# ucla-vision/xivo

Measured on AMD Instinct MI355X. Metric: EKF updates/sec (state dim 250, 80 feats) @1 GPU; % MFMA roofline, higher is better.
Workload: dtype f64; 1 GPU; MH gating + UpdateJosephForm: state dim 250, 80 features (M=160), XIVO row sparsity, P/H/inn/R resident in HBM; filters_per_gpu=16384, global_batch=16384, parallelism=replicas x1 (no collective), pipeline=sparse-H (row-pair compressed H, whitened in-solve Joseph form), hand_over=dense H -> row-pair compressed rows every step, inside the timed region, route=sparse_in_solve, not_spd_filters=0

## Files before the change

### xivo_amd/csrc/chol_trsm.hip

```cpp
#include <stdlib.h>

#include "mfma_util.h"
#include <stdio.h>

#include "trsm_lds_kernel.h"

namespace xivo_hip {

namespace {

__global__ __launch_bounds__(256) void fwd_vec_kernel(const double* __restrict__ LUall, long strideLU, int ldlu,
                                                     const double* __restrict__ invDall, long strideInvD,
                                                     const double* __restrict__ innall, long strideInn, double* __restrict__ yall,
                                                     long strideY, int Mp, int batch) {
  __shared__ double sy[4][384];
  const int wv = threadIdx.x >> 6;
  const int filt = blockIdx.x * (blockDim.x >> 6) + wv;
  if (filt >= batch) return;
  const int lane = threadIdx.x & 63, r = lane & 15, part = lane >> 4;
  const double* L = LUall + (long)filt * strideLU;
  const double* invD = invDall + (long)filt * strideInvD;
  const double* inn = innall + (long)filt * strideInn;
  double* y = yall + (long)filt * strideY;
  double* ys = sy[wv];
  const int nb = Mp / 16;
  for (int k = 0; k < nb; ++k) {
    double acc = 0.0;
    for (int c = part; c < 16 * k; c += 4) acc = fma(L[(16 * k + r) + (long)c * ldlu], ys[c], acc);
    acc += __shfl_xor(acc, 16);
    acc += __shfl_xor(acc, 32);
    const double rhs = inn[16 * k + r] - acc;
    double out = 0.0;
#pragma unroll
    for (int c = 0; c < 16; ++c) out = fma(invD[(long)k * 512 + r + 16 * c], __shfl(rhs, c), out);
    if (part == 0) { ys[16 * k + r] = out; y[16 * k + r] = out; }
  }
}


template <int NBM>
__global__ __launch_bounds__(1024) void pnew_reg_f64_kernel(PnewRegArgs g) {
  extern __shared__ __attribute__((aligned(16))) double sL[];
  const int bidx = blockIdx.x;
  const int filt = (bidx >> 3) * 8 + (bidx & 7);
  if (filt >= g.batch) return;
  if (g.skip_status && g.skip_status[filt] != 0) return;
  const int tid = threadIdx.x, lane = tid & 63, wave = __builtin_amdgcn_readfirstlane(tid >> 6);
  const int li = lane & 15, lg = lane >> 4;
  const int nb = g.Mp / 16;
  const int c0 = wave * 16;
  const bool live = c0 < g.Np;
  const double* __restrict__ G = g.G + (long)filt * g.strideG;
  d4 X[NBM];
#pragma unroll
  for (int i = 0; i < NBM; ++i) {
    X[i] = d4{0.0, 0.0, 0.0, 0.0};
    if (live && i < nb) {
#pragma unroll
      for (int r = 0; r < 4; ++r) X[i][r] = G[(c0 + li) + (long)(16 * i + lg + 4 * r) * g.ldg];
    }
  }
  sym_tiles_from_regs<NBM>(X, X, sL, g.K + (long)filt * g.strideK, g.ldk, g.T + (long)filt * g.strideT, g.ldt,
                           g.P + (long)filt * g.strideP, g.ldp, nb, g.Np / 16, g.jbp, live, wave, wave, lane);
}

template <int NBM, int WH, int NWS = 8>
__global__ __launch_bounds__(64 * NWS, NWS == 8 ? (NBM <= 4 ? 6 : (NBM <= 8 ? 4 : 2)) : 2) void trsm_stream_f64_kernel(TrsmArgs g) {
  extern __shared__ __attribute__((aligned(16))) double sL[];
  constexpr int PSZ = (NBM + 1) * 256;
  constexpr int WCOLS = 16 * NWS;
  const int chunks = (g.Np + WCOLS - 1) / WCOLS;
  const int b = blockIdx.x;
  const int xcd = b & 7, slot = b >> 3;
  const int filt = (slot / chunks) * 8 + xcd;
  const int chunk = slot % chunks;
  if (filt >= g.batch) return;
  const int tid = threadIdx.x, lane = tid & 63, wave = __builtin_amdgcn_readfirstlane(tid >> 6);
  const int li = lane & 15, lg = lane >> 4;
  const int nb = g.Mp / 16;
  const double* __restrict__ LU = g.LU + (long)filt * g.strideLU;
  const double* __restrict__ invD = g.invD + (long)filt * g.strideInvD;
  const long ld = g.ldlu;
  const int c0 = chunk * WCOLS + wave * 16;
  const bool live = c0 < g.Np;
  const __amdgpu_buffer_rsrc_t rPHT = buf_rsrc(g.PHT + (long)filt * g.stridePHT), rK = buf_rsrc(g.K + (long)filt * g.strideK),
                               rInn = buf_rsrc(g.fwd_only ? g.y + (long)filt * g.strideY : g.inn + (long)filt * g.strideInn),
                               rY = buf_rsrc(WH ? g.Yout + (long)filt * g.strideY2 : g.K);
  const unsigned vPHT = (unsigned)((live ? c0 + li : 0) + lg * g.ldpht) * 8u;
  const unsigned vK = (unsigned)((live ? c0 + li : 0) + lg * g.ldk) * 8u;
  const unsigned vY = WH ? (unsigned)((live ? c0 + li : 0) + lg * g.ldy2) * 8u : 0u;

  d4 X[NBM];
#pragma unroll
  for (int i = 0; i < NBM; ++i) {
    X[i] = d4{0.0, 0.0, 0.0, 0.0};
    if (live && i < nb) {
#pragma unroll
      for (int r = 0; r < 4; ++r) X[i][r] = buf_ld(rPHT, vPHT, (unsigned)((16 * i + 4 * r) * g.ldpht) * 8u);
    }
  }

  auto issue_panel = [&](int k, bool fwd, double* buf) {
    const int j0 = fwd ? k : 0, nj = (fwd ? nb - k : k + 1) + ((WH && !fwd) ? 1 : 0);
    for (int q = wave; q < nj * 2; q += NWS) {
      int j = j0 + (q >> 1);
      const int h = q & 1;
      const bool extra = WH && !fwd && (q >> 1) == nj - 1;
      const double* src;
      if (extra) { j = nb; src = LU + (16 * k + 2 * (lane & 7)) + (long)(16 * k + 8 * h + (lane >> 3)) * ld; }
      else if (j == k) src = invD + (long)k * 512 + (fwd ? 0 : 256) + h * 128 + 2 * lane;
      else src = LU + (16 * j + 2 * (lane & 7)) + (long)(16 * k + 8 * h + (lane >> 3)) * ld;
      __builtin_amdgcn_global_load_lds((const __attribute__((address_space(1))) void*)src,
                                       (__attribute__((address_space(3))) void*)(buf + j * 256 + h * 128), 16, 0, 0);
    }
  };
  double* buf0 = sL;
  double* buf1 = sL + PSZ;

  issue_panel(0, true, buf0);
#pragma unroll
  for (int k = 0; k < NBM; ++k) {
    if (k < nb) {
      asm volatile("s_waitcnt vmcnt(0)" ::: "memory");
      __syncthreads();
      const double* cur = (k & 1) ? buf1 : buf0;
      if (k + 1 < nb) issue_panel(k + 1, true, (k & 1) ? buf0 : buf1);
      if (live) {
        d4 t = d4{0.0, 0.0, 0.0, 0.0};
#pragma unroll
        for (int s = 0; s < 4; ++s) t = mfma(cur[k * 256 + li + 16 * (4 * s + lg)], X[k][s], t);
        X[k] = t;
#pragma unroll
        for (int s = 0; s < 4; ++s) {
#pragma unroll
          for (int i = k + 1; i < NBM; ++i) {
            if (i < nb) X[i] = mfma(-cur[i * 256 + li + 16 * (4 * s + lg)], t[s], X[i]);
          }
        }
      }
      __builtin_amdgcn_sched_barrier(0);
    }
  }
  double part = 0.0;
  if (WH && live) {
#pragma unroll
    for (int i = 0; i < NBM; ++i) {
      if (i < nb) {
#pragma unroll
        for (int r = 0; r < 4; ++r) buf_st(X[i][r], rK, vK, (unsigned)((16 * i + 4 * r) * g.ldk) * 8u);
      }
      __builtin_amdgcn_sched_barrier(0);
    }
  }
  __syncthreads();
  if (!g.fwd_only) issue_panel(nb - 1, false, buf0);
  int par = 0;
#pragma unroll
  for (int k = NBM - 1; k >= 0; --k) {
    if (k < nb && !g.fwd_only) {
      asm volatile("s_waitcnt vmcnt(0)" ::: "memory");
      __syncthreads();
      const double* cur = par ? buf1 : buf0;
      if (k > 0) issue_panel(k - 1, false, par ? buf0 : buf1);
      par ^= 1;
      if (live) {
        d4 wk = d4{0.0, 0.0, 0.0, 0.0};
        if (WH) {
          if (k == nb - 1) wk = X[k];
          else {
#pragma unroll
            for (int r = 0; r < 4; ++r) wk[r] = buf_ld(rK, vK, (unsigned)((16 * k + 4 * r) * g.ldk) * 8u);
          }
        }
        d4 t = d4{0.0, 0.0, 0.0, 0.0};
#pragma unroll
        for (int s = 0; s < 4; ++s) t = mfma(cur[k * 256 + li + 16 * (4 * s + lg)], X[k][s], t);
        if (WH) {
#pragma unroll
          for (int s2 = 0; s2 < 4; ++s2) {
            const int kk = 4 * s2 + lg;
            const double a = cur[nb * 256 + li + 16 * kk];
            X[k] = mfma(kk >= li ? -a : 0.0, t[s2], X[k]);
          }
#pragma unroll
          for (int r = 0; r < 4; ++r) part = fma(t[r], buf_ld(rInn, (unsigned)lg * 8u, (unsigned)(16 * k + 4 * r) * 8u), part);
        } else {
          X[k] = t;
        }
#pragma unroll
        for (int s = 0; s < 4; ++s) {
#pragma unroll
          for (int i = 0; i < k; ++i) X[i] = mfma(-cur[i * 256 + li + 16 * (4 * s + lg)], t[s], X[i]);
        }
        if (WH) {
#pragma unroll
          for (int r = 0; r < 4; ++r) {
            if (g.out_f32) buf_st_f32((float)(wk[r] + X[k][r]), rY, vY >> 1, (unsigned)((16 * k + 4 * r) * g.ldy2) * 4u);
            else buf_st(wk[r] + X[k][r], rY, vY, (unsigned)((16 * k + 4 * r) * g.ldy2) * 8u);
          }
          X[k] = wk - X[k];
        }
      }
      __builtin_amdgcn_sched_barrier(0);
    }
  }
  if (!live) return;
#pragma unroll
  for (int i = 0; i < NBM; ++i) {
    if (i < nb) {
#pragma unroll
      for (int r = 0; r < 4; ++r) {
        if (WH && g.out_f32) buf_st_f32((float)X[i][r], rY, vY >> 1, (unsigned)(g.Np * g.Mp + (16 * i + 4 * r) * g.ldy2) * 4u);
        else buf_st(X[i][r], rK, vK, (unsigned)((16 * i + 4 * r) * g.ldk) * 8u);
        if (!WH) part = fma(X[i][r], buf_ld(rInn, (unsigned)lg * 8u, (unsigned)(16 * i + 4 * r) * 8u), part);
      }
    }
    __builtin_amdgcn_sched_barrier(0);
  }
  part += __shfl_xor(part, 16);
  part += __shfl_xor(part, 32);
  if (lg == 0) g.err[(long)filt * g.strideErr + c0 + li] = part;
}

template <int NBM, int WH, int NWS = 8>
int launch_trsm_stream_t(const TrsmArgs& g, hipStream_t stream) {
  const int chunks = (g.Np + 16 * NWS - 1) / (16 * NWS);
  const int grid = ((g.batch + 7) / 8) * 8 * chunks;
  const size_t lds = (size_t)2 * (NBM + 1) * 256 * sizeof(double);
  static bool attr_set = false;
  if (!attr_set) {
    (void)hipFuncSetAttribute(reinterpret_cast<const void*>(&trsm_stream_f64_kernel<NBM, WH, NWS>), hipFuncAttributeMaxDynamicSharedMemorySize, 160 * 1024);
    attr_set = true;
  }
  hipLaunchKernelGGL((trsm_stream_f64_kernel<NBM, WH, NWS>), dim3(grid), dim3(64 * NWS), lds, stream, g);
  return (int)hipGetLastError();
}
static int stream_capacity(int nb, bool whitened) {
  if (whitened && nb <= 8) return nb <= 4 ? 4 : (nb <= 6 ? 6 : 8);
  if (nb <= 14) return 14;
  if (whitened) return nb <= 19 ? 19 : (nb <= 22 ? 22 : 24);
  return nb <= 16 ? 16 : (nb <= 22 ? 22 : 24);
}

template <int NBM, int TF>
int launch_trsm_lds_tf(const TrsmArgs& g_in, hipStream_t stream) {
  TrsmArgs g = g_in;
  const int nb = g.Mp / 16;
  const int chunks = (g.Np + 255) / 256;
  const int grid = ((g.batch + 7) / 8) * 8 * chunks;
  size_t lds = (size_t)nb * (nb + 1) / 2 * 16 * 17 * sizeof(double);
  if (TF) {
    lds = 160 * 1024;
    g.t_jbp = (int)(lds / 2 / ((size_t)nb * 4 * 64 * sizeof(double)));
    if (g.t_jbp > 16) g.t_jbp = 16;
  }
  static bool attr_set = false;
  if (!attr_set) {
    (void)hipFuncSetAttribute(reinterpret_cast<const void*>(&trsm_lds_f64_kernel<NBM, TF>),
                              hipFuncAttributeMaxDynamicSharedMemorySize, 160 * 1024);
    attr_set = true;
  }
  hipLaunchKernelGGL((trsm_lds_f64_kernel<NBM, TF>), dim3(grid), dim3(1024), lds, stream, g);
  return (int)hipGetLastError();
}
template <int NBM>
int launch_trsm_lds_t(const TrsmArgs& g, hipStream_t stream) {
  if (g.Yout && !g.fwd_only) return launch_trsm_lds_tf<NBM, 5>(g, stream);
  {
    if (g.T && trsm_forms_T(g.Mp, g.Np))
      return g.fwd_only ? launch_trsm_lds_tf<NBM, 2>(g, stream)
                        : (g.joseph ? launch_trsm_lds_tf<NBM, 4>(g, stream) : launch_trsm_lds_tf<NBM, 1>(g, stream));
  }
  return launch_trsm_lds_tf<NBM, 0>(g, stream);
}

}

bool pnew_reg_supported(int Mp, int Np) {
  return Mp / 16 <= 10 && Np <= 256 && Np % 16 == 0;
}

template <int NBM>
static int launch_pnew_reg_t(const PnewRegArgs& g_in, hipStream_t stream) {
  PnewRegArgs g = g_in;
  const int nb = g.Mp / 16;
  const size_t lds = 160 * 1024;
  g.jbp = (int)(lds / 2 / ((size_t)nb * 4 * 64 * sizeof(double)));
  if (g.jbp > 16) g.jbp = 16;
  static bool attr_set = false;
  if (!attr_set) {
    (void)hipFuncSetAttribute(reinterpret_cast<const void*>(&pnew_reg_f64_kernel<NBM>),
                              hipFuncAttributeMaxDynamicSharedMemorySize, 160 * 1024);
    attr_set = true;
  }
  hipLaunchKernelGGL((pnew_reg_f64_kernel<NBM>), dim3(((g.batch + 7) / 8) * 8), dim3(1024), lds, stream, g);
  return (int)hipGetLastError();
}

int launch_pnew_reg_f64(const PnewRegArgs& g, hipStream_t stream) {
  if (g.batch <= 0) return 0;
  const int nb = g.Mp / 16;
  if (nb <= 6) return launch_pnew_reg_t<6>(g, stream);
  if (nb <= 10) return launch_pnew_reg_t<10>(g, stream);
  return (int)hipErrorInvalidValue;
}

void pnew_reg_kernel_label(int Mp, char* buf, size_t n) { snprintf(buf, n, "pnew_reg_f64_kernel<%d>", Mp / 16 <= 6 ? 6 : 10); }

bool trsm_latency_route(int Mp, int batch) { return Mp / 16 <= 14 && batch <= 64; }

bool trsm_forms_T(int Mp, int Np) {
  return Mp / 16 <= 11 && Np <= 256 && Np % 16 == 0;
}

int launch_trsm_f64(const TrsmArgs& g, hipStream_t stream) {
  if (g.batch <= 0) return 0;
  const int nb = g.Mp / 16;
  if (g.latency && g.Yout && !g.fwd_only && nb <= 14) {
    if (nb <= 4) return launch_trsm_stream_t<4, 1, 4>(g, stream);
    if (nb <= 6) return launch_trsm_stream_t<6, 1, 4>(g, stream);
    if (nb <= 8) return launch_trsm_stream_t<8, 1, 4>(g, stream);
    return launch_trsm_stream_t<14, 1, 4>(g, stream);
  }
  if (g.stream8 && g.Yout && !g.fwd_only && nb <= 8) {
    if (nb <= 4) return launch_trsm_stream_t<4, 1>(g, stream);
    if (nb <= 6) return launch_trsm_stream_t<6, 1>(g, stream);
    return launch_trsm_stream_t<8, 1>(g, stream);
  }
  if (g.out_f32 && g.Yout && !g.fwd_only && nb <= 14) return launch_trsm_stream_t<14, 1>(g, stream);
  if (nb <= 6) return launch_trsm_lds_t<6>(g, stream);
  if (nb <= 10) return launch_trsm_lds_t<10>(g, stream);
  if (nb <= 11 && !(g.Yout && !g.fwd_only)) return launch_trsm_lds_t<11>(g, stream);
  const bool wh = g.Yout && !g.fwd_only;
  if (nb <= 24) {
    switch (stream_capacity(nb, wh) * 2 + (wh ? 1 : 0)) {
      case 14 * 2: return launch_trsm_stream_t<14, 0>(g, stream);
      case 14 * 2 + 1: return launch_trsm_stream_t<14, 1>(g, stream);
      case 16 * 2: return launch_trsm_stream_t<16, 0>(g, stream);
      case 19 * 2 + 1: return launch_trsm_stream_t<19, 1>(g, stream);
      case 22 * 2: return launch_trsm_stream_t<22, 0>(g, stream);
      case 22 * 2 + 1: return launch_trsm_stream_t<22, 1>(g, stream);
      case 24 * 2: return launch_trsm_stream_t<24, 0>(g, stream);
      default: return launch_trsm_stream_t<24, 1>(g, stream);
    }
  }
  return (int)hipErrorInvalidValue;
}

int launch_fwd_vec(const double* LU, long strideLU, int ldlu, const double* invD, long strideInvD, const double* inn, long strideInn,
                   double* y, long strideY, int Mp, int batch, hipStream_t stream) {
  if (batch <= 0) return 0;
  hipLaunchKernelGGL(fwd_vec_kernel, dim3((batch + 3) / 4), dim3(256), 0, stream, LU, strideLU, ldlu, invD, strideInvD, inn, strideInn,
                     y, strideY, Mp, batch);
  return (int)hipGetLastError();
}

void trsm_kernel_label(int Mp, char* buf, size_t n, int forms_T, bool latency, bool stream8) {
  const int nb = Mp / 16;
  if (latency && forms_T == 5 && nb <= 14) snprintf(buf, n, "trsm_stream_f64_kernel<%d,1,4>", stream_capacity(nb, true));
  else if (stream8 && forms_T >= 4 && nb <= 8) snprintf(buf, n, "trsm_stream_f64_kernel<%d,1>", stream_capacity(nb, true));
  else if (nb <= 11) snprintf(buf, n, "trsm_lds_f64_kernel<%d,%d>", nb <= 6 ? 6 : (nb <= 10 ? 10 : 11), forms_T);
  else snprintf(buf, n, "trsm_stream_f64_kernel<%d,%d>", stream_capacity(nb, forms_T >= 4), forms_T >= 4 ? 1 : 0);
}

}
```

### xivo_amd/csrc/trsm_lds_kernel.h

```cpp
#pragma once
#include <stdlib.h>
#include <stdio.h>

#include "mfma_util.h"

#ifndef XIVO_TRACE
#define XIVO_TRACE 0
#endif
#if XIVO_TRACE
__device__ unsigned long long xivo_trace_buf[512 * 32];
__device__ unsigned long long xivo_trace2_buf[128 * 16 * 4 * 16];
#define XTR(i) do { if (T4 && !WOUT && threadIdx.x == 0 && (blockIdx.x & 63) == 0 && (blockIdx.x >> 6) < 512) \
    xivo_trace_buf[(blockIdx.x >> 6) * 32 + (i)] = __builtin_amdgcn_s_memtime(); } while (0)
#define XTRP(i) do { if (threadIdx.x == 0 && (blockIdx.x & 63) == 0 && (blockIdx.x >> 6) < 512) \
    xivo_trace_buf[(blockIdx.x >> 6) * 32 + (i)] = __builtin_amdgcn_s_memtime(); } while (0)
#define XTR2(ph, slot) do { if ((threadIdx.x & 63) == 0 && (blockIdx.x & 63) == 0 && (blockIdx.x >> 6) < 128 && (ph) < 4 && (slot) < 16) \
    xivo_trace2_buf[(((blockIdx.x >> 6) * 16 + (threadIdx.x >> 6)) * 4 + (ph)) * 16 + (slot)] = __builtin_amdgcn_s_memtime(); } while (0)
extern "C" int xivo_hip_debug_read_trace(unsigned long long* out, int n) {
  return (int)hipMemcpyFromSymbol(out, HIP_SYMBOL(xivo_trace_buf), (size_t)n * sizeof(unsigned long long));
}
extern "C" int xivo_hip_debug_read_trace2(unsigned long long* out, int n) {
  return (int)hipMemcpyFromSymbol(out, HIP_SYMBOL(xivo_trace2_buf), (size_t)n * sizeof(unsigned long long));
}
#else
#define XTR(i) do {} while (0)
#define XTRP(i) do {} while (0)
#define XTR2(ph, slot) do {} while (0)
#endif

namespace xivo_hip {

namespace {

typedef unsigned int bufu2 __attribute__((ext_vector_type(2)));
__device__ __forceinline__ __amdgpu_buffer_rsrc_t buf_rsrc(const void* p) {
  return __builtin_amdgcn_make_buffer_rsrc(const_cast<void*>(p), 0, 0x7FFFFFFF, 0x00020000);
}
__device__ __forceinline__ double buf_ld(__amdgpu_buffer_rsrc_t r, unsigned voff, unsigned soff) {
  return __builtin_bit_cast(double, __builtin_amdgcn_raw_buffer_load_b64(r, voff, soff, 0));
}
__device__ __forceinline__ double buf_ld_once(__amdgpu_buffer_rsrc_t r, unsigned voff, unsigned soff) {
  return __builtin_bit_cast(double, __builtin_amdgcn_raw_buffer_load_b64(r, voff, soff, 0));
}
__device__ __forceinline__ void buf_st_f32(float v, __amdgpu_buffer_rsrc_t r, unsigned voff, unsigned soff) {
  __builtin_amdgcn_raw_buffer_store_b32(__builtin_bit_cast(unsigned, v), r, voff, soff, 0);
}
__device__ __forceinline__ void buf_st(double v, __amdgpu_buffer_rsrc_t r, unsigned voff, unsigned soff) {
  __builtin_amdgcn_raw_buffer_store_b64(__builtin_bit_cast(bufu2, v), r, voff, soff, 0);
}
__device__ __forceinline__ void buf_st_out(double v, __amdgpu_buffer_rsrc_t r, unsigned voff, unsigned soff) {
  __builtin_amdgcn_raw_buffer_store_b64(__builtin_bit_cast(bufu2, v), r, voff, soff, 0);
}

template <int NBM, bool SRC_REGS = false, bool NEG_OUT = false, bool YREGS = false, int NWV = 16>
__device__ __forceinline__ void sym_tiles_from_regs(const d4 (&X)[NBM], const d4 (&Wr)[NBM], double* sL, const double* __restrict__ Src, int ldsrc,
                                                    const double* __restrict__ Minit, int ldm, double* __restrict__ Out, int ldo,
                                                    int nb, int nwl, int jbp, bool live, int w, int wave, int lane) {
  const int li = lane & 15, lg = lane >> 4;
  const int nph = (nwl + jbp - 1) / jbp;
  const int bufsz = jbp * nb * 256;
  auto issue = [&](int p) {
    const int jb0 = p * jbp, nj = min(jbp, nwl - jb0);
    double* buf = sL + (p & 1) * bufsz;
    if (SRC_REGS) {
      if (live && w >= jb0 && w < jb0 + nj) {
        double* dst = buf + (w - jb0) * nb * 256 + lane;
#pragma unroll
        for (int mb = 0; mb < NBM; ++mb) {
          if (mb < nb) {
#pragma unroll
            for (int r = 0; r < 4; ++r) dst[(mb * 4 + r) * 64] = YREGS ? fma(2.0, Wr[mb][r], -X[mb][r]) : X[mb][r];
          }
        }
      }
      return;
    }
    for (int q = wave; q < nj * 2 * nb; q += NWV) {
      const int jl = q / (2 * nb), t = q - jl * 2 * nb;
      const double* src = Src + (16 * (jb0 + jl) + 2 * (lane & 7)) + (long)(8 * t + (lane >> 3)) * ldsrc;
      __builtin_amdgcn_global_load_lds((const __attribute__((address_space(1))) void*)src,
                                       (__attribute__((address_space(3))) void*)(buf + jl * nb * 256 + t * 128), 16, 0, 0);
    }
  };
  auto my_tiles = [&](int p) -> unsigned {
    unsigned todo = 0;
    if (!live || p >= nph) return todo;
    const int jb0 = p * jbp, nj = min(jbp, nwl - jb0);
    for (int jl = 0; jl < nj; ++jl) {
      int d = w - (jb0 + jl);
      if (d < 0) d += nwl;
      if (2 * d < nwl || (2 * d == nwl && w > jb0 + jl)) todo |= 1u << jl;
    }
    return todo;
  };
  const __amdgpu_buffer_rsrc_t rM = buf_rsrc(Minit), rO = buf_rsrc(Out);
  const unsigned vM = (unsigned)(li + lg * ldm) * 8u;
  const unsigned vO = (unsigned)(li + lg * ldo) * 8u, vOt = (unsigned)(lg + li * ldo) * 8u;
  auto load_m = [&](int jb, d4& acc) {
    const int ba = jb <= w ? w : jb, bb = jb <= w ? jb : w;
#pragma unroll
    for (int r = 0; r < 4; ++r)
      acc[r] = buf_ld_once(rM, vM, (unsigned)(16 * ba + (16 * bb + 4 * r) * ldm) * 8u);
  };
  issue(0);
  unsigned todo = my_tiles(0);
  d4 nxt = d4{0.0, 0.0, 0.0, 0.0};
  if (todo) load_m(__builtin_ctz(todo), nxt);
  for (int p = 0; p < nph; ++p) {
    asm volatile("s_waitcnt vmcnt(0)" ::: "memory");
    __syncthreads();
    const int jb0 = p * jbp;
    const double* buf = sL + (p & 1) * bufsz;
    bool fetch = p + 1 < nph;
    while (todo) {
      const int jl = __builtin_ctz(todo);
      todo &= todo - 1;
      const int jb = jb0 + jl;
      d4 acc = -nxt;
      if (fetch) { asm volatile("" : "+v"(acc[0]), "+v"(acc[1]), "+v"(acc[2]), "+v"(acc[3])); issue(p + 1); fetch = false; }
      if (todo) load_m(jb0 + __builtin_ctz(todo), nxt);
      const double* Bop = buf + jl * nb * 256 + lane;
      if (jb <= w) {
#pragma unroll
        for (int mb = 0; mb < NBM; ++mb) {
          if (mb < nb) {
#pragma unroll
            for (int r = 0; r < 4; ++r) acc = mfma(Bop[(mb * 4 + r) * 64], X[mb][r], acc);
          }
        }
      } else {
#pragma unroll
        for (int mb = 0; mb < NBM; ++mb) {
          if (mb < nb) {
#pragma unroll
            for (int r = 0; r < 4; ++r) acc = mfma(X[mb][r], Bop[(mb * 4 + r) * 64], acc);
          }
        }
      }
      const int ba = jb <= w ? w : jb, bbk = jb <= w ? jb : w;
      const int a = 16 * ba + li, b = 16 * bbk + lg;
#pragma unroll
      for (int r = 0; r < 4; ++r) {
        const int bb = b + 4 * r;
        if (jb != w || a >= bb) {
          const double v = NEG_OUT ? -acc[r] : acc[r];
          buf_st_out(v, rO, vO, (unsigned)(16 * ba + (16 * bbk + 4 * r) * ldo) * 8u);
          if (a != bb) buf_st_out(v, rO, vOt, (unsigned)(16 * bbk + 4 * r + 16 * ba * ldo) * 8u);
        }
      }
    }
    if (fetch) issue(p + 1);
    todo = my_tiles(p + 1);
    if (todo) load_m((p + 1) * jbp + __builtin_ctz(todo), nxt);
  }
}

template <int NBM, int NWV>
__device__ __forceinline__ void whitened_tiles_from_stash(d4 (&X)[NBM], double* sL, const double* __restrict__ Src, int ldsrc,
                                                          double* __restrict__ Pio, int ldp, int nb, int nwl, int jbp, bool live,
                                                          int w, int wave, int lane) {
  const int li = lane & 15, lg = lane >> 4;
  const int nph = (nwl + jbp - 1) / jbp;
  const int bufsz = jbp * nb * 256;
  const int gw = w / jbp;
  auto issue = [&](int p) {
    const int jb0 = p * jbp, nj = min(jbp, nwl - jb0);
    double* buf = sL + (p & 1) * bufsz;
    for (int q = wave; q < nj * 2 * nb; q += NWV) {
      const int jl = q / (2 * nb), t = q - jl * 2 * nb;
      const double* src = Src + (16 * (jb0 + jl) + 2 * (lane & 7)) + (long)(8 * t + (lane >> 3)) * ldsrc;
      __builtin_amdgcn_global_load_lds((const __attribute__((address_space(1))) void*)src,
                                       (__attribute__((address_space(3))) void*)(buf + jl * nb * 256 + t * 128), 16, 0, 0);
    }
  };
  auto my_tiles = [&](int p) -> unsigned {
    if (!live || p >= nph || gw > p) return 0u;
    const int jb0 = p * jbp, nj = min(jbp, nwl - jb0);
    if (gw < p) return (1u << nj) - 1u;
    unsigned todo = 0;
    for (int jl = 0; jl < nj; ++jl) {
      int d = w - (jb0 + jl);
      if (d < 0) d += nj;
      if (2 * d < nj || (2 * d == nj && w > jb0 + jl)) todo |= 1u << jl;
    }
    return todo;
  };
  const __amdgpu_buffer_rsrc_t rP = buf_rsrc(Pio);
  const unsigned vP = (unsigned)(li + lg * ldp) * 8u, vPt = (unsigned)(lg + li * ldp) * 8u;
  auto load_m = [&](int jb, d4& acc) {
    const int ba = jb <= w ? w : jb, bb = jb <= w ? jb : w;
#pragma unroll
    for (int r = 0; r < 4; ++r)
      acc[r] = buf_ld_once(rP, vP, (unsigned)(16 * ba + (16 * bb + 4 * r) * ldp) * 8u);
  };
  issue(0);
  unsigned todo = my_tiles(0);
  d4 nxt = d4{0.0, 0.0, 0.0, 0.0};
  if (todo) load_m(__builtin_ctz(todo), nxt);
  for (int p = 0; p < nph; ++p) {
    XTRP(8 + 3 * p);
    asm volatile("s_waitcnt vmcnt(0)" ::: "memory");
    XTRP(9 + 3 * p);
    __syncthreads();
    XTRP(10 + 3 * p);
    XTR2(p, 0);
    int tslot = 2;
    const int jb0 = p * jbp;
    const double* buf = sL + (p & 1) * bufsz;
    if (live && gw == p) {
      double* dst = sL + (p & 1) * bufsz + (w - jb0) * nb * 256 + lane;
#pragma unroll
      for (int mb = 0; mb < NBM; ++mb) {
        if (mb < nb) {
#pragma unroll
          for (int r = 0; r < 4; ++r) {
            const double wv = dst[(mb * 4 + r) * 64];
            const double v = wv - X[mb][r];
            X[mb][r] = fma(2.0, wv, -v);
            dst[(mb * 4 + r) * 64] = v;
          }
        }
      }
    }
    lds_barrier();
    XTR2(p, 1);
    bool fetch = p + 1 < nph;
    while (todo) {
      const int jl = __builtin_ctz(todo);
      todo &= todo - 1;
      const int jb = jb0 + jl;
      d4 acc = -nxt;
      if (fetch) { asm volatile("" : "+v"(acc[0]), "+v"(acc[1]), "+v"(acc[2]), "+v"(acc[3])); issue(p + 1); fetch = false; }
      if (todo) load_m(jb0 + __builtin_ctz(todo), nxt);
      const double* Bop = buf + jl * nb * 256 + lane;
      if (jb < w) {
#pragma unroll
        for (int mb = 0; mb < NBM; ++mb) {
          if (mb < nb) {
#pragma unroll
            for (int r = 0; r < 4; ++r) acc = mfma(Bop[(mb * 4 + r) * 64], X[mb][r], acc);
          }
        }
      } else {
#pragma unroll
        for (int mb = 0; mb < NBM; ++mb) {
          if (mb < nb) {
#pragma unroll
            for (int r = 0; r < 4; ++r) acc = mfma(X[mb][r], Bop[(mb * 4 + r) * 64], acc);
          }
        }
      }
      XTR2(p, tslot); ++tslot;
      const int ba = jb <= w ? w : jb, bbk = jb <= w ? jb : w;
      const int a = 16 * ba + li, b = 16 * bbk + lg;
#pragma unroll
      for (int r = 0; r < 4; ++r) {
        const int bb = b + 4 * r;
        if (jb != w || a >= bb) {
          const double v = -acc[r];
          buf_st_out(v, rP, vP, (unsigned)(16 * ba + (16 * bbk + 4 * r) * ldp) * 8u);
          if (a != bb) buf_st_out(v, rP, vPt, (unsigned)(16 * bbk + 4 * r + 16 * ba * ldp) * 8u);
        }
      }
      XTR2(p, tslot); ++tslot;
    }
    XTR2(p, 14);
    if (fetch) issue(p + 1);
    todo = my_tiles(p + 1);
    if (todo) load_m((p + 1) * jbp + __builtin_ctz(todo), nxt);
  }
  XTRP(8 + 3 * nph);
}

template <int NBM, int TF, int NWV = 16, int MINB = 1>
__global__ __launch_bounds__(64 * NWV, MINB) void trsm_lds_f64_kernel(TrsmArgs g) {
  constexpr int BLK = 16 * 17;
  constexpr int NT = 64 * NWV;
  static_assert(TF != 3, "TF == 3 (the round-2 expanded Joseph form) was removed in round 6");
  constexpr bool T4 = TF == 4 || TF == 5;
  constexpr bool WOUT = TF == 5;
  constexpr bool KEEPW = T4 && (NBM <= 6 || (NBM == 7 && NWV <= 12 && MINB <= 3));
  constexpr bool PACK = T4 && NBM > 10;
  constexpr bool DREGS = T4 && !KEEPW && !WOUT;
  extern __shared__ __attribute__((aligned(16))) double sL[];
  const int chunks = (g.Np + 16 * NWV - 1) / (16 * NWV);
  const int b = blockIdx.x;
  const int xcd = b & 7, slot = b >> 3;
  const int filt = (slot / chunks) * 8 + xcd;
  const int chunk = slot % chunks;
  if (filt >= g.batch) return;
  const int tid = threadIdx.x, lane = tid & 63, wave = __builtin_amdgcn_readfirstlane(tid >> 6);
  const int li = lane & 15, lg = lane >> 4;
  const int nb = g.Mp / 16;
  const double* __restrict__ LU = g.LU + (long)filt * g.strideLU;
  const double* __restrict__ invD = g.invD + (long)filt * g.strideInvD;
  const double* __restrict__ PHT = g.PHT + (long)filt * g.stridePHT;
  const long ld = g.ldlu;

  XTR(0);
  const int c0 = chunk * 16 * NWV + wave * 16;
  const bool live = c0 < g.Np;
  const __amdgpu_buffer_rsrc_t rPHT = buf_rsrc(PHT), rK = buf_rsrc(g.K + (long)filt * g.strideK),
                               rInn = buf_rsrc(g.fwd_only ? g.y + (long)filt * g.strideY : g.inn + (long)filt * g.strideInn);
  const unsigned vPHT = (unsigned)((c0 + li) + lg * g.ldpht) * 8u;
  const unsigned vK = (unsigned)((c0 + li) + lg * g.ldk) * 8u;
  d4 X[NBM];
  auto load_rhs = [&](int i0, int i1) {
#pragma unroll
    for (int i = 0; i < NBM; ++i) {
      if (i >= i0 && i < i1) {
        X[i] = d4{0.0, 0.0, 0.0, 0.0};
        if (live && i < nb) {
#pragma unroll
          for (int r = 0; r < 4; ++r) X[i][r] = buf_ld_once(rPHT, vPHT, (unsigned)((16 * i + 4 * r) * g.ldpht) * 8u);
        }
      }
    }
  };
  load_rhs(0, NBM);
  d4 Wk[KEEPW ? NBM : 1];
#pragma unroll
  for (int i = 0; i < (KEEPW ? NBM : 1); ++i) Wk[i] = d4{0.0, 0.0, 0.0, 0.0};

  const int nblk = nb * (nb + 1) / 2;
  constexpr bool DIAG = !PACK && T4;
  constexpr int CPY = (NBM * (NBM + 1) / 2 * 128 + NT - 1) / NT;
  constexpr int CPD = DIAG ? (NBM * 128 + NT - 1) / NT : 0;
  constexpr int CPB = 4;
  double* sD = sL + nblk * BLK;
#pragma unroll
  for (int u0 = 0; u0 < CPY + CPD; u0 += CPB) {
    d2 cv[CPB], cu[CPB];
#pragma unroll
    for (int q = 0; q < CPB; ++q) {
      const int u = u0 + q;
      cv[q] = d2{0.0, 0.0}; cu[q] = d2{0.0, 0.0};
      if (u < CPY) {
        const int e = tid + NT * u;
        if (e < nblk * 128) {
          const int t = e >> 7, w = e & 127;
          int i = 0;
          while ((i + 1) * (i + 2) / 2 <= t) ++i;
          const int k = t - i * (i + 1) / 2;
          const int r = (w & 7) * 2, c = w >> 3;
          cv[q] = *reinterpret_cast<const d2*>(i != k ? LU + (16 * i + r) + (long)(16 * k + c) * ld : invD + (long)k * 512 + r + 16 * c);
          if (PACK && i == k) { cu[q][0] = LU[(16 * k + c) + (long)(16 * k + r) * ld]; cu[q][1] = LU[(16 * k + c) + (long)(16 * k + r + 1) * ld]; }
        }
      } else if (u < CPY + CPD) {
        const int e = tid + NT * (u - CPY);
        if (e < nb * 128) {
          const int k = e >> 7, w = e & 127;
          cv[q] = *reinterpret_cast<const d2*>(LU + (16 * k + (w & 7) * 2) + (long)(16 * k + (w >> 3)) * ld);
        }
      }
    }
#pragma unroll
    for (int q = 0; q < CPB; ++q) {
      const int u = u0 + q;
      if (u < CPY) {
        const int e = tid + NT * u;
        if (e < nblk * 128) {
          const int t = e >> 7, w = e & 127;
          int i = 0;
          while ((i + 1) * (i + 2) / 2 <= t) ++i;
          const int k = t - i * (i + 1) / 2;
          const int r = (w & 7) * 2, c = w >> 3;
          d2 v = cv[q];
          if (PACK && i == k) { v[0] = r >= c ? v[0] : cu[q][0]; v[1] = r + 1 >= c ? v[1] : cu[q][1]; }
          sL[t * BLK + r + 17 * c] = v[0];
          sL[t * BLK + r + 1 + 17 * c] = v[1];
        }
      } else if (u < CPY + CPD) {
        const int e = tid + NT * (u - CPY);
        if (e < nb * 128) {
          const int k = e >> 7, w = e & 127;
          const int r = (w & 7) * 2, c = w >> 3;
          sD[k * BLK + r + 17 * c] = r >= c ? cv[q][0] : 0.0;
          sD[k * BLK + r + 1 + 17 * c] = r + 1 >= c ? cv[q][1] : 0.0;
        }
      }
    }
    __builtin_amdgcn_sched_barrier(0);
  }
  if (PACK) {
    for (int e = tid; e < nb * 16; e += NT) {
      const int k = e >> 4, c = e & 15;
      sL[(k * (k + 1) / 2 + k) * BLK + 16 + 17 * c] = LU[(16 * k + c) + (long)(16 * k + c) * ld];
    }
  }
  XTR(1);
  __syncthreads();
  XTR(2);
  if (!TF && !live) return;
  if (live) {
#pragma unroll
  for (int k = 0; k < NBM; ++k) {
    if (k < nb) {
      const double* Dk = sL + (k * (k + 1) / 2 + k) * BLK;
      d4 t = d4{0.0, 0.0, 0.0, 0.0};
#pragma unroll
      for (int s = 0; s < 4; ++s) {
        double a = Dk[li + 17 * (4 * s + lg)];
        if (PACK) a = li >= 4 * s + lg ? a : 0.0;
        t = mfma(a, X[k][s], t);
      }
      X[k] = t;
#pragma unroll
      for (int s = 0; s < 4; ++s) {
#pragma unroll
        for (int i = k + 1; i < NBM; ++i) {
          if (i < nb) {
            const double a = sL[(i * (i + 1) / 2 + k) * BLK + li + 17 * (4 * s + lg)];
            X[i] = mfma(-a, t[s], X[i]);
          }
        }
      }
    }
  }
  XTR(3);
  double part = 0.0;
  if (KEEPW) {
#pragma unroll
    for (int i = 0; i < NBM; ++i) Wk[i] = X[i];
  }
  if (T4 && !KEEPW) {
#pragma unroll
    for (int i = 0; i < NBM; ++i) {
      if (i < nb) {
#pragma unroll
        for (int r = 0; r < 4; ++r) buf_st(X[i][r], rK, vK, (unsigned)((16 * i + 4 * r) * g.ldk) * 8u);
      }
    }
  }
  XTR(4);
#pragma unroll
  for (int k = NBM - 1; k >= 0; --k) {
    if (k < nb && !g.fwd_only) {
      const double* Dk = sL + (k * (k + 1) / 2 + k) * BLK;
      d4 wk = d4{0.0, 0.0, 0.0, 0.0};
      if (KEEPW) wk = Wk[k];
      else if (T4 && !DREGS) {
        if (k == nb - 1) wk = X[k];
        else {
#pragma unroll
          for (int r = 0; r < 4; ++r) wk[r] = buf_ld(rK, vK, (unsigned)((16 * k + 4 * r) * g.ldk) * 8u);
        }
      }
      d4 t = d4{0.0, 0.0, 0.0, 0.0};
#pragma unroll
      for (int s = 0; s < 4; ++s) {
        double a = Dk[(4 * s + lg) + 17 * li];
        if (PACK) a = 4 * s + lg >= li ? a : 0.0;
        t = mfma(a, X[k][s], t);
      }
      if (T4) {
        const double* Lk = PACK ? Dk : sD + k * BLK;
#pragma unroll
        for (int s2 = 0; s2 < 4; ++s2) {
          const int kk = 4 * s2 + lg;
          if (PACK) {
            const double a = Lk[kk > li ? li + 17 * kk : 16 + 17 * li];
            X[k] = mfma(kk >= li ? -a : 0.0, t[s2], X[k]);
          } else {
            X[k] = mfma(-Lk[kk + 17 * li], t[s2], X[k]);
          }
        }
#pragma unroll
        for (int r = 0; r < 4; ++r) part = fma(t[r], buf_ld(rInn, (unsigned)lg * 8u, (unsigned)(16 * k + 4 * r) * 8u), part);
      } else {
        X[k] = t;
      }
#pragma unroll
      for (int s = 0; s < 4; ++s) {
#pragma unroll
        for (int i = 0; i < k; ++i) {
          const double a = sL[(k * (k + 1) / 2 + i) * BLK + (4 * s + lg) + 17 * li];
          X[i] = mfma(-a, t[s], X[i]);
        }
      }
      if (T4) {
        if (WOUT) {
          const __amdgpu_buffer_rsrc_t rY = buf_rsrc(g.Yout + (long)filt * g.strideY2);
#pragma unroll
          for (int r = 0; r < 4; ++r) buf_st(wk[r] + X[k][r], rY, (unsigned)((c0 + li) + lg * g.ldy2) * 8u, (unsigned)((16 * k + 4 * r) * g.ldy2) * 8u);
        }
        if (!DREGS) X[k] = wk - X[k];
        __builtin_amdgcn_sched_barrier(0);
      }
    }
  }

  if (!T4) {
#pragma unroll
    for (int i = 0; i < NBM; ++i) {
      if (i < nb) {
#pragma unroll
        for (int r = 0; r < 4; ++r) {
          if (TF != 2) buf_st(X[i][r], rK, vK, (unsigned)((16 * i + 4 * r) * g.ldk) * 8u);
          part = fma(X[i][r], buf_ld(rInn, (unsigned)lg * 8u, (unsigned)(16 * i + 4 * r) * 8u), part);
        }
      }
    }
  }
  part += __shfl_xor(part, 16);
  part += __shfl_xor(part, 32);
  if (lg == 0) g.err[(long)filt * g.strideErr + c0 + li] = part;


  }
  if (!TF) return;

  XTR(5);
  __syncthreads();
  XTR(6);
  if (T4) {
    if (WOUT) {
      if (live) {
#pragma unroll
        for (int i = 0; i < NBM; ++i) {
          if (i < nb) {
#pragma unroll
            for (int r = 0; r < 4; ++r) buf_st(X[i][r], rK, vK, (unsigned)((16 * i + 4 * r) * g.ldk) * 8u);
          }
        }
      }
      return;
    }
    if (g.skip_status && g.skip_status[filt] != 0) return;
    double* Pio = g.T + (long)filt * g.strideT;
    if constexpr (KEEPW) sym_tiles_from_regs<NBM, true, true, true, NWV>(X, Wk, sL, nullptr, 0, Pio, g.ldt, Pio, g.ldt, nb, g.Np / 16, g.t_jbp,
                                                                 live, c0 >> 4, wave, lane);
    else whitened_tiles_from_stash<NBM, NWV>(X, sL, g.K + (long)filt * g.strideK, g.ldk, Pio, g.ldt, nb, g.Np / 16, g.t_jbp, live, c0 >> 4, wave, lane);
    return;
  }
  if (TF == 2) {
    if (g.skip_status && g.skip_status[filt] != 0) return;
    double* Pio = g.T + (long)filt * g.strideT;
    sym_tiles_from_regs<NBM, true, true, false, NWV>(X, X, sL, nullptr, 0, Pio, g.ldt, Pio, g.ldt, nb, g.Np / 16, g.t_jbp, live, c0 >> 4, wave, lane);
    return;
  }
  sym_tiles_from_regs<NBM, false, false, false, NWV>(X, X, sL, PHT, g.ldpht, g.Pm + (long)filt * g.stridePm, g.ldpm, g.T + (long)filt * g.strideT, g.ldt,
                           nb, g.Np / 16, g.t_jbp, live, c0 >> 4, wave, lane);
}

}

}
```

Before: 997,400 updates/s.

## Add full-shape TRSM kernel variant with pre-negated LDS factors and LDS-staged innovation

Adds a compile-time FULL specialization of the whitened Joseph-form TRSM kernel, used when the block count equals NBM (10 or 11, i.e. M=160). It fixes nb at compile time, stores the off-diagonal L blocks and D blocks pre-negated in LDS so MFMA operands skip a negate, and stages the innovation vector in LDS instead of reloading it through buffer loads. It also adds scheduling barriers and an opaque lane copy to steer register allocation. The cost is extra instantiations and one more LDS region, and the sign flips have to be applied consistently on every path that reads sL/sD.

```diff
diff --git a/xivo_amd/csrc/chol_trsm.hip b/xivo_amd/csrc/chol_trsm.hip
--- a/xivo_amd/csrc/chol_trsm.hip
+++ b/xivo_amd/csrc/chol_trsm.hip
@@ -242,10 +242,15 @@
   return nb <= 16 ? 16 : (nb <= 22 ? 22 : 24);
 }
 
-template <int NBM, int TF>
+static bool solve_generic_forced() { static const bool on = getenv("XIVO_HIP_SOLVE_GENERIC") != nullptr; return on; }
+
+template <int NBM, int TF, bool FULL = false>
 int launch_trsm_lds_tf(const TrsmArgs& g_in, hipStream_t stream) {
   TrsmArgs g = g_in;
   const int nb = g.Mp / 16;
+  if constexpr (!FULL && TF == 4 && (NBM == 10 || NBM == 11)) {
+    if (nb == NBM && !solve_generic_forced()) return launch_trsm_lds_tf<NBM, TF, true>(g_in, stream);
+  }
   const int chunks = (g.Np + 255) / 256;
   const int grid = ((g.batch + 7) / 8) * 8 * chunks;
   size_t lds = (size_t)nb * (nb + 1) / 2 * 16 * 17 * sizeof(double);
@@ -256,11 +261,11 @@
   }
   static bool attr_set = false;
   if (!attr_set) {
-    (void)hipFuncSetAttribute(reinterpret_cast<const void*>(&trsm_lds_f64_kernel<NBM, TF>),
+    (void)hipFuncSetAttribute(reinterpret_cast<const void*>(&trsm_lds_f64_kernel<NBM, TF, 16, 1, FULL>),
                               hipFuncAttributeMaxDynamicSharedMemorySize, 160 * 1024);
     attr_set = true;
   }
-  hipLaunchKernelGGL((trsm_lds_f64_kernel<NBM, TF>), dim3(grid), dim3(1024), lds, stream, g);
+  hipLaunchKernelGGL((trsm_lds_f64_kernel<NBM, TF, 16, 1, FULL>), dim3(grid), dim3(1024), lds, stream, g);
   return (int)hipGetLastError();
 }
 template <int NBM>
diff --git a/xivo_amd/csrc/trsm_lds_kernel.h b/xivo_amd/csrc/trsm_lds_kernel.h
--- a/xivo_amd/csrc/trsm_lds_kernel.h
+++ b/xivo_amd/csrc/trsm_lds_kernel.h
@@ -155,10 +155,11 @@
   }
 }
 
-template <int NBM, int NWV>
+template <int NBM, int NWV, bool FULL = false>
 __device__ __forceinline__ void whitened_tiles_from_stash(d4 (&X)[NBM], double* sL, const double* __restrict__ Src, int ldsrc,
-                                                          double* __restrict__ Pio, int ldp, int nb, int nwl, int jbp, bool live,
+                                                          double* __restrict__ Pio, int ldp, int nb_rt, int nwl, int jbp, bool live,
                                                           int w, int wave, int lane) {
+  const int nb = FULL ? NBM : nb_rt;
   const int li = lane & 15, lg = lane >> 4;
   const int nph = (nwl + jbp - 1) / jbp;
   const int bufsz = jbp * nb * 256;
@@ -233,6 +234,9 @@
       if (fetch) { asm volatile("" : "+v"(acc[0]), "+v"(acc[1]), "+v"(acc[2]), "+v"(acc[3])); issue(p + 1); fetch = false; }
       if (todo) load_m(jb0 + __builtin_ctz(todo), nxt);
       const double* Bop = buf + jl * nb * 256 + lane;
+      int lane2 = lane;
+      if (FULL) asm volatile("" : "+v"(lane2));
+      const double* Bop2 = buf + jl * nb * 256 + lane2;
       if (jb < w) {
 #pragma unroll
         for (int mb = 0; mb < NBM; ++mb) {
@@ -246,7 +250,7 @@
         for (int mb = 0; mb < NBM; ++mb) {
           if (mb < nb) {
 #pragma unroll
-            for (int r = 0; r < 4; ++r) acc = mfma(X[mb][r], Bop[(mb * 4 + r) * 64], acc);
+            for (int r = 0; r < 4; ++r) acc = mfma(X[mb][r], Bop2[(mb * 4 + r) * 64], acc);
           }
         }
       }
@@ -272,11 +276,12 @@
   XTRP(8 + 3 * nph);
 }
 
-template <int NBM, int TF, int NWV = 16, int MINB = 1>
+template <int NBM, int TF, int NWV = 16, int MINB = 1, bool FULL = false>
 __global__ __launch_bounds__(64 * NWV, MINB) void trsm_lds_f64_kernel(TrsmArgs g) {
   constexpr int BLK = 16 * 17;
   constexpr int NT = 64 * NWV;
   static_assert(TF != 3, "TF == 3 (the round-2 expanded Joseph form) was removed in round 6");
+  static_assert(!FULL || (TF == 4 && NBM >= 8), "the full-shape form is that of the in-kernel product off the stash");
   constexpr bool T4 = TF == 4 || TF == 5;
   constexpr bool WOUT = TF == 5;
   constexpr bool KEEPW = T4 && (NBM <= 6 || (NBM == 7 && NWV <= 12 && MINB <= 3));
@@ -291,7 +296,7 @@
   if (filt >= g.batch) return;
   const int tid = threadIdx.x, lane = tid & 63, wave = __builtin_amdgcn_readfirstlane(tid >> 6);
   const int li = lane & 15, lg = lane >> 4;
-  const int nb = g.Mp / 16;
+  const int nb = FULL ? NBM : g.Mp / 16;
   const double* __restrict__ LU = g.LU + (long)filt * g.strideLU;
   const double* __restrict__ invD = g.invD + (long)filt * g.strideInvD;
   const double* __restrict__ PHT = g.PHT + (long)filt * g.stridePHT;
@@ -328,6 +333,10 @@
   constexpr int CPD = DIAG ? (NBM * 128 + NT - 1) / NT : 0;
   constexpr int CPB = 4;
   double* sD = sL + nblk * BLK;
+  constexpr bool INN_LDS = DREGS;
+  double* sInn = sL + (nblk + (DIAG ? nb : 0)) * BLK;
+  double innv = 0.0;
+  if (INN_LDS && tid < 16 * nb) innv = buf_ld(rInn, (unsigned)tid * 8u, 0u);
 #pragma unroll
   for (int u0 = 0; u0 < CPY + CPD; u0 += CPB) {
     d2 cv[CPB], cu[CPB];
@@ -367,16 +376,16 @@
           const int r = (w & 7) * 2, c = w >> 3;
           d2 v = cv[q];
           if (PACK && i == k) { v[0] = r >= c ? v[0] : cu[q][0]; v[1] = r + 1 >= c ? v[1] : cu[q][1]; }
-          sL[t * BLK + r + 17 * c] = v[0];
-          sL[t * BLK + r + 1 + 17 * c] = v[1];
+          sL[t * BLK + r + 17 * c] = i != k ? -v[0] : v[0];
+          sL[t * BLK + r + 1 + 17 * c] = i != k ? -v[1] : v[1];
         }
       } else if (u < CPY + CPD) {
         const int e = tid + NT * (u - CPY);
         if (e < nb * 128) {
           const int k = e >> 7, w = e & 127;
           const int r = (w & 7) * 2, c = w >> 3;
-          sD[k * BLK + r + 17 * c] = r >= c ? cv[q][0] : 0.0;
-          sD[k * BLK + r + 1 + 17 * c] = r + 1 >= c ? cv[q][1] : 0.0;
+          sD[k * BLK + r + 17 * c] = r >= c ? -cv[q][0] : -0.0;
+          sD[k * BLK + r + 1 + 17 * c] = r + 1 >= c ? -cv[q][1] : -0.0;
         }
       }
     }
@@ -388,6 +397,7 @@
       sL[(k * (k + 1) / 2 + k) * BLK + 16 + 17 * c] = LU[(16 * k + c) + (long)(16 * k + c) * ld];
     }
   }
+  if (INN_LDS && tid < 16 * nb) sInn[tid] = innv;
   XTR(1);
   __syncthreads();
   XTR(2);
@@ -411,10 +421,11 @@
         for (int i = k + 1; i < NBM; ++i) {
           if (i < nb) {
             const double a = sL[(i * (i + 1) / 2 + k) * BLK + li + 17 * (4 * s + lg)];
-            X[i] = mfma(-a, t[s], X[i]);
-          }
-        }
-      }
+            X[i] = mfma(a, t[s], X[i]);
+          }
+        }
+      }
+      if (FULL) __builtin_amdgcn_sched_barrier(0);
     }
   }
   XTR(3);
@@ -462,11 +473,11 @@
             const double a = Lk[kk > li ? li + 17 * kk : 16 + 17 * li];
             X[k] = mfma(kk >= li ? -a : 0.0, t[s2], X[k]);
           } else {
-            X[k] = mfma(-Lk[kk + 17 * li], t[s2], X[k]);
-          }
-        }
-#pragma unroll
-        for (int r = 0; r < 4; ++r) part = fma(t[r], buf_ld(rInn, (unsigned)lg * 8u, (unsigned)(16 * k + 4 * r) * 8u), part);
+            X[k] = mfma(Lk[kk + 17 * li], t[s2], X[k]);
+          }
+        }
+#pragma unroll
+        for (int r = 0; r < 4; ++r) part = fma(t[r], INN_LDS ? sInn[16 * k + 4 * r + lg] : buf_ld(rInn, (unsigned)lg * 8u, (unsigned)(16 * k + 4 * r) * 8u), part);
       } else {
         X[k] = t;
       }
@@ -475,7 +486,7 @@
 #pragma unroll
         for (int i = 0; i < k; ++i) {
           const double a = sL[(k * (k + 1) / 2 + i) * BLK + (4 * s + lg) + 17 * li];
-          X[i] = mfma(-a, t[s], X[i]);
+          X[i] = mfma(a, t[s], X[i]);
         }
       }
       if (T4) {
@@ -530,7 +541,7 @@
     double* Pio = g.T + (long)filt * g.strideT;
     if constexpr (KEEPW) sym_tiles_from_regs<NBM, true, true, true, NWV>(X, Wk, sL, nullptr, 0, Pio, g.ldt, Pio, g.ldt, nb, g.Np / 16, g.t_jbp,
                                                                  live, c0 >> 4, wave, lane);
-    else whitened_tiles_from_stash<NBM, NWV>(X, sL, g.K + (long)filt * g.strideK, g.ldk, Pio, g.ldt, nb, g.Np / 16, g.t_jbp, live, c0 >> 4, wave, lane);
+    else whitened_tiles_from_stash<NBM, NWV, FULL>(X, sL, g.K + (long)filt * g.strideK, g.ldk, Pio, g.ldt, nb, g.Np / 16, g.t_jbp, live, c0 >> 4, wave, lane);
     return;
   }
   if (TF == 2) {
```

Measured after the change: 1.019 million updates/s (median of 6 runs). 2.2% higher.
